# Chang-Tun-Yu/HLS-final-Visual-Odometry

Hardware: AMD Instinct MI355X
Metric: stereo frame-pairs/sec (detect+match), KITTI 1241x376; matches bit-exact (higher is better)
Workload: dtype u8; 1 GPU; KITTI 1241x376 stereo quad-match (prev/curr x L/R), default 50x50 bins; noise=0, gpu_max_hw_queues=4, streams_per_gpu=256, frames_in_hbm=8, parallelism=1x independent stream groups

## Files before the change

### hls-final-visual-odometry_amd/csrc/engine.hip

```cpp
#include "engine.h"

namespace vh_engine {

thread_local std::string t_last_error;

VhMatchArgs Group::role_args() const {
  VhMatchArgs a{};
  a.S = S; a.pair_cur = pairs(); a.rows = S;
  if (seq) {
    a.rows = seq_n;
    a.seq_prev_last = std::max(seq_n_prev - 1, 0);
    a.seq_lo = seq_first == 0 ? 1 : 0;
    a.seq_void = 2 * VH_RING * S;
  }
  return a;
}

int32_t Group::sync_all() {
  VH_HIP(hipStreamSynchronize(stream));
  VH_HIP(hipStreamSynchronize(match_stream));
  VH_HIP(hipStreamSynchronize(post_stream));
  VH_HIP(hipStreamSynchronize(down_stream));
  for (int k = 0; k < kVoteStreams; k++) if (vote_stream[k]) VH_HIP(hipStreamSynchronize(vote_stream[k]));
  if (sparse) { const int32_t rs = sparse->sync_all(); if (rs) return rs; }
// ... 93 lines not shown

  sets = VhSets{};
  sets.cap = cap;
  sets.binsize = p.match_binsize;
  sets.inv_binsize = p.match_binsize > 32768 ? 0u : (uint32_t)(((1ull << 32) + p.match_binsize - 1) / p.match_binsize);
  sets.ubn = (dims[0] + p.match_binsize - 1) / p.match_binsize;
  sets.vbn = (dims[1] + p.match_binsize - 1) / p.match_binsize;
  sets.nbins = 4 * sets.ubn * sets.vbn;
  sets.max_tiles = cap / VH_TILE_Q + 5;
  sets.W = dims[0]; sets.H = dims[1];
  {
    const int32_t blk = g.scale * (g.n + 1);
    const int64_t per_axis = (p.match_binsize + blk - 1) / blk + 1;
    sets.stage_cap = (int32_t)std::min<int64_t>(per_axis * per_axis, cap);
  }
  const size_t ns = n_sets();
  if ((rc = dmalloc(&sets.feat, ns * cap * 12, false))) return rc;
  if ((rc = dmalloc(&sets.f_uv, ns * cap, false))) return rc;
  if ((rc = dmalloc(&sets.s_uv, ns * cap, false))) return rc;
  if ((rc = dmalloc(&sets.s_idx, ns * cap, false))) return rc;
  if ((rc = dmalloc(&sets.s_desc, ns * cap * 8, false))) return rc;
  if ((rc = dmalloc(&sets.bin_start, ns * (sets.nbins + 1), true))) return rc;
  if ((rc = dmalloc(&sets.hist, ns * sets.nbins, true))) return rc;
  if ((rc = dmalloc(&sets.cursor, ns * sets.nbins, true))) return rc;
  if ((rc = dmalloc(&sets.tmp_idx, ns * cap, false))) return rc;
  if ((rc = dmalloc(&sets.stage, ns * (size_t)sets.nbins * sets.stage_cap, false))) return rc;
  if ((rc = dmalloc(&sets.count, ns, true))) return rc;
  const size_t nrow = 4 * (size_t)dims[1];
  if ((rc = dmalloc(&sets.row_start, ns * (nrow + 1), true))) return rc;
  if ((rc = dmalloc(&sets.row_hist, ns * nrow, true))) return rc;
  if ((rc = dmalloc(&sets.row_cursor, ns * nrow, true))) return rc;
  if ((rc = dmalloc(&sets.r_pos, ns * cap, false))) return rc;
  if ((rc = dmalloc(&sets.tiles, ns * sets.max_tiles, false))) return rc;
  if ((rc = dmalloc(&sets.tile_cnt, ns, true))) return rc;
  if ((rc = dmalloc(&sets.check, 4, true))) return rc;
  if ((rc = dmalloc(&det.d_rec, 2 * (size_t)S * std::max(g.nblocks, 1), false))) return rc;
  if ((rc = dmalloc(&det.d_chunk_count, 2 * (size_t)S * g.nchunks, true))) return rc;
  for (int k = 0; k < 2; k++) {
    if ((rc = dmalloc(&mt.d_best2[k], 4 * (size_t)S * cap, false))) return rc;
    if ((rc = dmalloc(&mt.d_chain2[k], 2 * (size_t)S * cap, false))) return rc;
  }
  mt.d_best = mt.d_best2[0]; mt.d_chain = mt.d_chain2[0];
  for (int k = 0; k < 2; k++) {
    if ((rc = dmalloc(&mt.d_mchunk2[k], (size_t)S * ((cap + 255) / 256), true))) return rc;
    VH_HIP(mt.h_out[k].alloc((size_t)S, hipHostMallocMapped));
    memset(mt.h_out[k], 0, sizeof(int4) * (size_t)S);
  }
  if ((rc = dmalloc(&mt.d_redo, 2 * (size_t)S, true))) return rc;
  if ((rc = dmalloc((uint8_t **)&mt.d_matches, (size_t)S * mcap * sizeof(vh_p_match), false))) return rc;
  if ((rc = dmalloc(&mt.d_match_count, (size_t)S, true))) return rc;
  if (serial && (size_t)S * mcap * sizeof(vh_p_match) <= (64u << 20)) {
    VH_HIP(mt.h_matches.alloc((size_t)S * mcap, hipHostMallocMapped));
  }
  if ((rc = dmalloc(&mt.d_overflow, (size_t)S, true))) return rc;
  VH_HIP(mt.h_overflow.alloc((size_t)S, hipHostMallocDefault));
  memset(mt.h_overflow, 0, sizeof(int32_t) * (size_t)S);
  if (p.half_resolution)
    if ((rc = dmalloc(&det.d_half, 2 * (size_t)S * g.bplm * g.Hm, false))) return rc;
  if (p.refinement > 0) {
    vh_refine_setup(rf);
    rf.W = dims[0]; rf.H = dims[1]; rf.bpl = dims[2];
    rf.pitch = round_up(dims[0], 16);
    rf.plane = (int64_t)rf.pitch * dims[1];
    rf.mode = p.refinement == 2 ? 2 : 1;
    const size_t nplanes = 2 * VH_RING * (size_t)S;
    if ((rc = dmalloc(&rf.du, nplanes * rf.plane, false))) return rc;
// ... 212 lines not shown
```

### hls-final-visual-odometry_amd/csrc/engine_api.hip

```cpp
#include "engine.h"

#include <mutex>
#include <thread>

namespace vh_engine {

#define ENTER(gq)                                   \
  if (!(gq)) return VH_ERR_INVALID_ARG;             \
  { hipError_t e_ = hipSetDevice((gq)->device);     \
    if (e_ != hipSuccess) { t_last_error = hipGetErrorString(e_); return VH_ERR_HIP; } }

struct Temp {
  Group *gq = nullptr;
  ~Temp() { if (gq) { (void)gq->sync_all(); delete gq; } }
};
int32_t temp_new(const vh_params *p, int32_t device, int32_t mf, int32_t mm, Temp &t) {
  if (!p) return VH_ERR_INVALID_ARG;
  vh_params q = *p;
  q.refinement = 0;
  return group_new(&q, device, 1, mf, mm, &t.gq);
}

struct EgoWork {
  std::mutex mu;
// ... 525 lines not shown
  return gq->get_features(0, which, out12, cap, n);
}
int32_t vh_host_alloc(int32_t device, size_t bytes, void **out) {
  if (!out || bytes == 0) return VH_ERR_INVALID_ARG;
  *out = nullptr;
  const int32_t rc = select_device(device);
  if (rc) return rc;
  VH_HIP(hipHostMalloc(out, bytes, hipHostMallocDefault));
  return VH_OK;
}
int32_t vh_host_free(void *ptr) {
  if (!ptr) return VH_OK;
  VH_HIP(hipHostFree(ptr));
  return VH_OK;
}
int32_t vh_synchronize(vh_matcher *m) { return vh_group_synchronize((vh_group *)m); }
int32_t vh_set_stream(vh_matcher *m, void *hip_stream) { return vh_group_set_stream((vh_group *)m, hip_stream); }
int32_t vh_clear_stream(vh_matcher *m) { return vh_group_clear_stream((vh_group *)m); }
int32_t vh_stream_wait_images(vh_matcher *m, void *hip_stream) { return vh_group_stream_wait_images((vh_group *)m, hip_stream); }

#ifdef VH_DEBUG_ROWS
int32_t vh_debug_rows(vh_matcher *m, int32_t which, int32_t *row_start, int32_t *r_pos, int32_t *bin_start) {
  Group *gq = (Group *)m; ENTER(gq);
  const int32_t set = vh_role_set(gq->S, gq->pairs(), 0, which);
  const size_t nrow = 4 * (size_t)gq->dims[1];
  VH_HIP(hipDeviceSynchronize());
  VH_HIP(hipMemcpy(row_start, gq->sets.row_start + (size_t)set * (nrow + 1), sizeof(int32_t) * (nrow + 1), hipMemcpyDeviceToHost));
  VH_HIP(hipMemcpy(r_pos, gq->sets.r_pos + (size_t)set * gq->cap, sizeof(int32_t) * gq->cap, hipMemcpyDeviceToHost));
  VH_HIP(hipMemcpy(bin_start, gq->sets.bin_start + (size_t)set * (gq->sets.nbins + 1), sizeof(int32_t) * (gq->sets.nbins + 1), hipMemcpyDeviceToHost));
  return gq->cap;
}
#endif

void vh_default_ego_params(vh_ego_params *e) {
  if (!e) return;
  memset(e, 0, sizeof(*e));
  e->ransac_iters = 200; e->reweighting = 1; e->inlier_threshold = 2.0;
  e->f = 1; e->cu = 0; e->cv = 0; e->base = 1;
}
int32_t vh_group_estimate_motion(vh_group *g, const vh_ego_params *e, const int32_t *rand3, double *tr, int32_t *ok,
                                 int32_t *n_inliers) {
  Group *gq = (Group *)g; ENTER(gq);
  return gq->estimate_motion(e, rand3, tr, ok, n_inliers);
}
int32_t vh_estimate_motion_stereo(const vh_ego_params *e, int32_t device, int32_t n_sets, const vh_p_match *pm,
                                  const int32_t *offsets, const int32_t *rand3, double *tr, int32_t *ok,
                                  int32_t *n_inliers, int32_t *inliers) {
  if (!e) return VH_ERR_INVALID_ARG;
  return estimate_stateless(device, n_sets, e->ransac_iters, 3, false, pm, offsets, rand3, tr, ok, n_inliers, inliers,
    [&](int64_t cap) { return sizeof(double) * 4 * (size_t)n_sets * (size_t)cap; },
    [&](const vh_p_match *d_pm, const int32_t *d_off, const int32_t *d_rand, uint8_t *d_scr, int64_t cap, double *d_tr, int32_t *d_ok, int32_t *d_inl) {
      vh_launch_ego(*e, n_sets, d_pm, 0, d_off, nullptr, 0, d_rand, (double *)d_scr, cap, d_tr, d_ok, d_ok + n_sets, d_inl, 0, nullptr);
    });
}

int32_t vh_group_post_begin(vh_group *g, int32_t cap_per_stream) {
  Group *gq = (Group *)g; ENTER(gq);
  return gq->post_begin(cap_per_stream);
}
int32_t vh_group_post_finish(vh_group *g, int32_t age, int32_t max_features, float bucket_width, float bucket_height, int32_t host_threads,
                             const vh_ego_params *e, const int32_t *rand3, double *tr, int32_t *ok, int32_t *n_inliers,
                             vh_p_match *bucketed, int32_t cap_per_stream, int32_t *counts, double *host_ms) {
  Group *gq = (Group *)g; ENTER(gq);
  if (host_threads < 1) host_threads = (int32_t)std::max(1u, std::thread::hardware_concurrency());
  return gq->post_finish(age, max_features, bucket_width, bucket_height, host_threads, e, rand3, nullptr, nullptr, tr, ok, n_inliers, bucketed, cap_per_stream, counts, host_ms);
}
// ... 330 lines not shown
```

### hls-final-visual-odometry_amd/csrc/kernels_bin.hip

```cpp
#include "vh_dev.h"
#include <algorithm>

#define VH_SCAN_T 256

namespace {

__device__ __forceinline__ int32_t bin_coord(int32_t x, int32_t binsize, int32_t nb) {
  return min(x / binsize, nb - 1);
}

__device__ __forceinline__ int32_t feature_bin(const int32_t *__restrict__ f, const VhSets &s) {
  const int32_t u = f[0], v = f[1], c = f[3];
  return (c * s.ubn + bin_coord(u, s.binsize, s.ubn)) * s.vbn + bin_coord(v, s.binsize, s.vbn);
}

__global__ void zero_counters_kernel(VhSets s, int32_t set0, int32_t nsets, int32_t *__restrict__ extra, int64_t n_extra) {
  const int64_t nb = (int64_t)nsets * s.nbins, nr = (int64_t)nsets * 4 * s.H;
  const int64_t total = 2 * nb + 2 * nr + nsets + n_extra;
  int32_t *hist = s.hist + (int64_t)set0 * s.nbins, *cur = s.cursor + (int64_t)set0 * s.nbins;
  int32_t *rh = s.row_hist + (int64_t)set0 * 4 * s.H, *rc = s.row_cursor + (int64_t)set0 * 4 * s.H;
  for (int64_t i = (int64_t)blockIdx.x * blockDim.x + threadIdx.x; i < total; i += (int64_t)gridDim.x * blockDim.x) {
    int64_t k = i;
    if (k < nb) { hist[k] = 0; continue; }
    k -= nb;
// ... 31 lines not shown

template <int EPT, class Load, class Emit>
__device__ __forceinline__ int32_t scan_exclusive(int32_t n, int32_t *sWave, Load load, Emit emit) {
  const int32_t tid = threadIdx.x, w = tid >> 6;
  int32_t carry = 0;
  for (int32_t b0 = 0; b0 < n; b0 += EPT * VH_SCAN_T) {
    const int32_t b = b0 + EPT * tid;
    int32_t v[EPT];
    int32_t mine = 0;
#pragma unroll
    for (int32_t k = 0; k < EPT; k++) { v[k] = (b + k < n) ? load(b + k) : 0; mine += v[k]; }
    const int32_t incl = scan_wave_inclusive(mine);
    if ((tid & 63) == 63) sWave[w] = incl;
    __syncthreads();
    int32_t before = 0, total = 0;
#pragma unroll
    for (int32_t k = 0; k < VH_SCAN_T / 64; k++) {
      const int32_t x = sWave[k];
      before += (k < w) ? x : 0;
      total += x;
    }
    int32_t run = carry + before + incl - mine;
#pragma unroll
    for (int32_t k = 0; k < EPT; k++) {
      if (b + k < n) emit(b + k, run, v[k]);
      run += v[k];
    }
    carry += total;
    __syncthreads();
  }
  return carry;
}

__device__ __forceinline__ void make_tiles(const VhSets &s, const int32_t *__restrict__ bs, int32_t set) {
  const int32_t span = s.ubn * s.vbn;
  int32_t tb[5];
  tb[0] = 0;
#pragma unroll
  for (int32_t c = 0; c < 4; c++) tb[c + 1] = tb[c] + (bs[(c + 1) * span] - bs[c * span] + VH_TILE_Q - 1) / VH_TILE_Q;
  int4 *__restrict__ tiles = s.tiles + (int64_t)set * s.max_tiles;
  for (int32_t i = threadIdx.x; i < 4 * s.ubn; i += VH_SCAN_T) {
    const int32_t c = i / s.ubn, col = i - c * s.ubn;
    const int32_t cls0 = bs[c * span], cls1 = bs[(c + 1) * span];
    const int32_t a = bs[(c * s.ubn + col) * s.vbn] - cls0, b = bs[(c * s.ubn + col + 1) * s.vbn] - cls0;
    for (int32_t t = (a + VH_TILE_Q - 1) / VH_TILE_Q; t * VH_TILE_Q < b; t++) {
      const int32_t k0 = cls0 + t * VH_TILE_Q, slot = tb[c] + t;
      if (slot < s.max_tiles) tiles[slot] = make_int4(k0, min(cls1, k0 + VH_TILE_Q), c, col);
    }
  }
  if (threadIdx.x == 0) s.tile_cnt[set] = min(tb[4], s.max_tiles);
}

__global__ void __launch_bounds__(VH_SCAN_T) bin_scan_kernel(VhSets s, int32_t set0) {
  __shared__ int32_t sWave[VH_SCAN_T / 64];
  const int32_t set = set0 + blockIdx.x, tid = threadIdx.x;
  VH_DET_SETPRIO();
  const int32_t *__restrict__ hist = s.hist + (int64_t)set * s.nbins;
  int32_t *__restrict__ bs = s.bin_start + (int64_t)set * (s.nbins + 1);
  const int32_t nfeat = scan_exclusive<4>(s.nbins, sWave, [&](int32_t b) { return hist[b]; },
                                       [&](int32_t b, int32_t prefix, int32_t) { bs[b] = prefix; });
  if (tid == 0) bs[s.nbins] = nfeat;
  __syncthreads();

  make_tiles(s, bs, set);

  const int32_t nrow = 4 * s.H;
  const int32_t *__restrict__ rh = s.row_hist + (int64_t)set * nrow;
  int32_t *__restrict__ rs = s.row_start + (int64_t)set * (nrow + 1);
  const int32_t nrowfeat = scan_exclusive<4>(nrow, sWave, [&](int32_t r) { return rh[r]; },
                                          [&](int32_t r, int32_t prefix, int32_t) { rs[r] = prefix; });
  if (tid == 0) rs[nrow] = nrowfeat;
}

__global__ void bin_fill_kernel(VhSets s, int32_t set0) {
  const int32_t set = set0 + blockIdx.y;
  const int32_t n = min(s.count[set], s.cap);
  for (int32_t i = blockIdx.x * blockDim.x + threadIdx.x; i < n; i += gridDim.x * blockDim.x) {
    const int32_t b = feature_bin(s.feat + ((int64_t)set * s.cap + i) * 12, s);
    const int32_t slot = s.bin_start[(int64_t)set * (s.nbins + 1) + b] + atomicAdd(&s.cursor[(int64_t)set * s.nbins + b], 1);
    s.tmp_idx[(int64_t)set * s.cap + slot] = i;
  }
}

__global__ void __launch_bounds__(256) bin_sort_kernel(VhSets s, int32_t set0, int32_t staged) {
  const int32_t set = set0 + blockIdx.y;
  const int32_t bin = blockIdx.x * 16 + (threadIdx.x >> 4), gl = threadIdx.x & 15;
  if (bin >= s.nbins) return;
  VH_DET_SETPRIO();
  const int32_t *__restrict__ bs = s.bin_start + (int64_t)set * (s.nbins + 1);
  const int32_t p0 = bs[bin], p1 = bs[bin + 1], L = p1 - p0;
  if (L <= 0) return;
#ifdef VH_CHECK
  if (staged && gl == 0) { int32_t len = L; VH_CHECK_RANGE(s, 6, len, 0, s.stage_cap + 1); }
#endif
  const int2 *__restrict__ stg = s.stage + ((int64_t)set * s.nbins + bin) * s.stage_cap - p0;
  const int32_t *__restrict__ tmp = s.tmp_idx + (int64_t)set * s.cap;
  const int32_t *__restrict__ feat = s.feat + (int64_t)set * s.cap * 12;
  int32_t *__restrict__ sidx = s.s_idx + (int64_t)set * s.cap;
  uint32_t *__restrict__ suv = s.s_uv + (int64_t)set * s.cap;
  uint4 *__restrict__ sdesc = (uint4 *)(s.s_desc + (int64_t)set * s.cap * 8);
  const int32_t nrow = 4 * s.H;
  const int32_t *__restrict__ rs = s.row_start + (int64_t)set * (nrow + 1);
  int32_t *__restrict__ rcur = s.row_cursor + (int64_t)set * nrow;
  int32_t *__restrict__ rpos = s.r_pos + (int64_t)set * s.cap;
  for (int32_t e0 = 0; e0 < L; e0 += 16) {
    const int32_t e = e0 + gl;
    int32_t mine = 0x7FFFFFFF, rowrel = 0;
    if (e < L) {
      if (staged) { const int2 m2 = stg[p0 + e]; mine = m2.x; rowrel = m2.y; }
      else mine = tmp[p0 + e];
    }
    uint4 h = make_uint4(0, 0, 0, 0), d0 = h, d1 = h;
    if (e < L) {
      const int32_t *f = feat + (int64_t)mine * 12;
      h = *(const uint4 *)f; d0 = *(const uint4 *)(f + 4); d1 = *(const uint4 *)(f + 8);
    }
    int32_t rank = 0;
    for (int32_t j0 = 0; j0 < L; j0 += 16) {
      const int32_t other = (j0 + gl < L) ? (staged ? stg[p0 + j0 + gl].x : tmp[p0 + j0 + gl]) : 0x7FFFFFFF;
      const int32_t m = min(16, L - j0);
      for (int32_t j = 0; j < m; j++) rank += (__shfl(other, j, 16) < mine) ? 1 : 0;
    }
    if (e < L) {
      const int32_t p = p0 + rank;
      sidx[p] = mine;
      suv[p] = (uint32_t)h.x | ((uint32_t)h.y << 16);
      sdesc[2 * (int64_t)p] = d0;
      sdesc[2 * (int64_t)p + 1] = d1;
      const int32_t row = (int32_t)h.w * s.H + (int32_t)h.y;
      int32_t rp = rs[row] + (staged ? rowrel : atomicAdd(&rcur[row], 1));
      VH_CHECK_RANGE(s, 4, rp, rs[row], rs[row + 1]);
      if (rp < rs[nrow]) rpos[rp] = p;
    }
  }
}

__global__ void ref_index_kernel(VhSets s, int32_t set, int32_t *__restrict__ bs_ref,
                                 int32_t *__restrict__ list_ref) {
  __shared__ int32_t sPos;
  const int32_t *__restrict__ bs = s.bin_start + (int64_t)set * (s.nbins + 1);
  const int32_t *__restrict__ sidx = s.s_idx + (int64_t)set * s.cap;
  if (threadIdx.x == 0) sPos = 0;
  __syncthreads();
  for (int32_t rb = 0; rb < s.nbins; rb++) {
    const int32_t ub = rb % s.ubn, vb = (rb / s.ubn) % s.vbn, c = rb / (s.ubn * s.vbn);
    const int32_t ib = (c * s.ubn + ub) * s.vbn + vb;
    const int32_t p0 = bs[ib], L = bs[ib + 1] - p0, pos = sPos;
    if (threadIdx.x == 0) bs_ref[rb] = pos;
    for (int32_t e = threadIdx.x; e < L; e += blockDim.x) list_ref[pos + e] = sidx[p0 + e];
    __syncthreads();
    if (threadIdx.x == 0) sPos = pos + L;
    __syncthreads();
  }
  if (threadIdx.x == 0) bs_ref[s.nbins] = sPos;
}

}

static int32_t feature_blocks(const VhSets &s) { return std::min(std::max(s.cap / 1024, 8), 256); }

void vh_launch_zero_counters(const VhSets &s, int32_t set0, int32_t nsets, int32_t *extra, int64_t n_extra, hipStream_t st) {
// ... 25 lines not shown
```

### hls-final-visual-odometry_amd/csrc/kernels_match.hip

```cpp
#include "vh_findmatch.h"
#include <algorithm>
#include <cstdlib>
#include <type_traits>

#ifdef VH_FLOW_STATS
__device__ unsigned long long g_flow_stats[12];
extern "C" int32_t vh_debug_flow_stats(unsigned long long *out, int32_t reset) {
  if (hipMemcpyFromSymbol(out, HIP_SYMBOL(g_flow_stats), sizeof(g_flow_stats)) != hipSuccess) return -3;
  if (reset) { unsigned long long z[12] = {0}; if (hipMemcpyToSymbol(HIP_SYMBOL(g_flow_stats), z, sizeof(z)) != hipSuccess) return -3; }
  return 0;
}
#define VH_STAT(k, n) do { if ((threadIdx.x & 63) == 0) atomicAdd(&g_flow_stats[k], (unsigned long long)(n)); } while (0)
#else
#define VH_STAT(k, n) do { } while (0)
#endif

#ifndef VH_MATCH_WAVES
#define VH_MATCH_WAVES 7
#endif
#ifndef VH_SNAKE
#define VH_SNAKE 1
#endif

namespace {

__device__ __forceinline__ int32_t wave_min(int32_t v) {
#pragma unroll
  for (int32_t d = 32; d >= 1; d >>= 1) v = min(v, __shfl_xor(v, d));
  return v;
}
__device__ __forceinline__ int32_t wave_max(int32_t v) {
#pragma unroll
  for (int32_t d = 32; d >= 1; d >>= 1) v = max(v, __shfl_xor(v, d));
  return v;
}

template <bool MAX>
__device__ __forceinline__ int32_t row16_allreduce(int32_t v) {
#define VH_ROW_STEP(CTRL)                                                                   \
  {                                                                                         \
    const int32_t t = __builtin_amdgcn_update_dpp(v, v, CTRL, 0xF, 0xF, false);             \
    v = MAX ? max(v, t) : min(v, t);                                                        \
  }
  VH_ROW_STEP(0x128)
  VH_ROW_STEP(0x124)
  VH_ROW_STEP(0x122)
  VH_ROW_STEP(0x121)
#undef VH_ROW_STEP
  return v;
}

template <class T>
__device__ __forceinline__ T ld_off(const T *base, uint32_t byte_off) { return *(const T *)((const char *)base + byte_off); }
template <class T>
// ... 253 lines not shown
                if (k < g.n) kk[k] = min(kk[k], tested_key_uniform_query(g.qd[k], g.lo2[k], span2, gu, g0, g1, (uint32_t)(pl - pbase)));
            });
        } else {
          const int32_t *__restrict__ crs = s.row_start + (int64_t)cset * (4 * s.H + 1);
          const int32_t *__restrict__ cpos = s.r_pos + (int64_t)cset * s.cap;
          const int32_t x0 = ld_uniform_i32(crs + c * s.H + max(g.vmin - rv, 0));
          const int32_t x1 = ld_uniform_i32(crs + c * s.H + min(g.vmax + rv, s.H - 1) + 1);
          for (int32_t x = x0 + lane; x < x1; x += 64) {
            int32_t cp = cpos[x];
            VH_CHECK_RANGE(s, 3, cp, pbase, pbase + pcnt);
            const uint32_t gu = cuv[cp];
            const uint4 g0 = cdesc[2 * (int64_t)cp], g1 = cdesc[2 * (int64_t)cp + 1];
#pragma unroll
            for (int32_t k = 0; k < VH_REDO_G; k++)
              if (k < g.n) kk[k] = min(kk[k], tested_key_uniform_query(g.qd[k], g.lo2[k], span2, gu, g0, g1, (uint32_t)(cp - pbase)));
          }
        }
#pragma unroll
        for (int32_t k = 0; k < VH_REDO_G; k++)
          if (k < g.n) {
            const uint64_t kf = wave_min_u64(kk[k]);
            int32_t wp = (int32_t)(uint32_t)kf;
            if (kf != ~0ull) VH_CHECK_RANGE(s, 7, wp, 0, pcnt);
            if (lane == g.lane[k]) res = kf == ~0ull ? -1 : pbase + wp;
          }
      }
    }
  }
  if (mine) st_off(tbl, (uint32_t)ld_off(qidx, (uint32_t)qpos * 4u) * 4u, res < 0 ? 0 : ld_off(cidx, (uint32_t)res * 4u));
}

template <int Q, int P, int KM, bool SPEC>
__device__ __forceinline__ void flow_tile(const VhSets &s, const VhMatchArgs &a, int32_t pass, int32_t stream,
                                          int32_t qset, int32_t cset, int32_t q0, int32_t q1, int32_t c, int32_t col0,
                                          int32_t pbase, int32_t pcnt, uint4 *wD, uint32_t *wU, TileOut<Q> &out) {
  constexpr int L = 64 / P;
  static_assert(L == 8 || L == 16, "every 16-lane row must hold the whole tile (row-wise window reduction)");
  constexpr int TRIP = 2 * P;
  const int32_t lane = threadIdx.x & 63, ph = lane / L, l = lane % L;
  const uint32_t *__restrict__ quv = s.s_uv + (int64_t)qset * s.cap;
  const uint4 *__restrict__ qdesc = (const uint4 *)(s.s_desc + (int64_t)qset * s.cap * 8);
  const uint32_t *__restrict__ cuv = s.s_uv + (int64_t)cset * s.cap;
  const uint4 *__restrict__ cdesc = (const uint4 *)(s.s_desc + (int64_t)cset * s.cap * 8);
  const int32_t *__restrict__ cbs = s.bin_start + (int64_t)cset * (s.nbins + 1);
  const int32_t rv = a.pass[pass].flow ? a.radius : a.disp_tol;

  bool (&valid)[Q] = out.valid;
  uint4 (&a0)[Q] = out.a0, (&a1)[Q] = out.a1;
  uint32_t (&uv1)[Q] = out.uv1;
  int32_t v_lo[Q];
  us2 lo2[Q];
  typedef typename KeyT<KM>::type key_t;
  const key_t KNONE = (key_t)~(key_t)0;
  key_t best_key[Q];
  int32_t umin = 0x7FFFFFFF, umax = -1, vmin = 0x7FFFFFFF, vmax = -1;
  int32_t (&qp)[Q] = out.qpos;
#pragma unroll
  for (int32_t qi = 0; qi < Q; qi++) {
    const int32_t q = q0 + L * qi + l;
    valid[qi] = q < q1;
    qp[qi] = valid[qi] ? q : q0;
  }
  {
    const int32_t *__restrict__ qbs = s.bin_start + (int64_t)qset * (s.nbins + 1);
    int32_t colb = col0, j = 0;
    int32_t csv = ld_off(qbs, (uint32_t)((c * s.ubn + min(colb + lane, s.ubn)) * s.vbn) * 4u);
    int32_t A = __builtin_amdgcn_readlane(csv, 0);
    int32_t k[Q];
#pragma unroll
    for (int32_t qi = 0; qi < Q; qi++) k[qi] = qp[qi];
    for (;;) {
      const int32_t B = __builtin_amdgcn_readlane(csv, j + 1);
      if (VH_SNAKE && ((colb + j) & 1)) {
#pragma unroll
        for (int32_t qi = 0; qi < Q; qi++) if (k[qi] >= A && k[qi] < B) qp[qi] = A + B - 1 - k[qi];
      }
      if (B >= q1 || colb + j + 1 >= s.ubn) break;
      A = B;
      if (++j == 63) { colb += 63; j = 0; csv = ld_off(qbs, (uint32_t)((c * s.ubn + min(colb + lane, s.ubn)) * s.vbn) * 4u); }
    }
  }
#pragma unroll
  for (int32_t qi = 0; qi < Q; qi++) {
    const int32_t ql = qp[qi];
    uv1[qi] = ld_off(quv, (uint32_t)ql * 4u);
    a0[qi] = ld_off(qdesc, (uint32_t)ql * 32u); a1[qi] = ld_off(qdesc, (uint32_t)ql * 32u + 16u);
    const int32_t u1 = uv1[qi] & 0xFFFF, v1 = uv1[qi] >> 16;
    v_lo[qi] = v1 - rv;
    lo2[qi] = window_lo2(uv1[qi], a.radius, rv);
    best_key[qi] = KNONE;
    umin = min(umin, u1); umax = max(umax, u1); vmin = min(vmin, v1); vmax = max(vmax, v1);
  }
  umin = __builtin_amdgcn_readfirstlane(row16_allreduce<false>(umin));
  umax = __builtin_amdgcn_readfirstlane(row16_allreduce<true>(umax));
  vmin = __builtin_amdgcn_readfirstlane(row16_allreduce<false>(vmin));
  vmax = __builtin_amdgcn_readfirstlane(row16_allreduce<true>(vmax));
  const VhBins ub = bins_of_interest(s, VhWindow{umin - a.radius, umax + a.radius, vmin - rv, vmax + rv});
  const int32_t UB0 = ub.ub0, UB1 = ub.ub1, VB0 = ub.vb0, VB1 = ub.vb1;
  const us2 span2 = window_span2(a.radius, rv);
  const int32_t ULO_MAX = umax - a.radius, UHI_MIN = umin + a.radius;
  const int32_t VLO_MAX = vmax - rv, VHI_MIN = vmin + rv;
  const int32_t VA0 = SPEC ? 0 : max(VB0, (max(VLO_MAX, 0) + s.binsize - 1) / s.binsize);
  const int32_t VA1 = SPEC ? 0 : min(VB1, (VHI_MIN + 1) / s.binsize - 1);

  auto make_key = [&](auto test, int32_t qi, uint32_t uv2, const uint4 &b0, const uint4 &b1, uint32_t seed) -> key_t {
    constexpr int TEST = decltype(test)::value;
    bool out = false;
    if (TEST == 2) {
      out = outside_window(uv2, lo2[qi], span2);
    } else if (TEST == 1) {
      out = (uint32_t)((int32_t)(uv2 >> 16) - v_lo[qi]) > (uint32_t)(2 * rv);
    }
    const key_t key = sad_key<KM>(a0[qi], a1[qi], b0, b1, seed);
    return (TEST != 0 && out) ? KNONE : key;
  };
  VH_STAT(0, 1); VH_STAT(5, q1 - q0); VH_STAT(6, UB1 - UB0 + 1);
  walk_region_lds<!SPEC>(s, cbs, cuv, cdesc, c, UB0, UB1, VB0, VB1, ULO_MAX, UHI_MIN, VA0, VA1, wD, wU,
    [&](int32_t pc, int32_t p1, int32_t pa0, int32_t pa1, const uint4 *cD, const uint32_t *cU) {
      VH_STAT(1, 1);
      const int32_t mcnt = min(64, p1 - pc);
      const int32_t jend = (mcnt + TRIP - 1) & ~(TRIP - 1);
      const uint4 *rd = cD + ph;
      const uint32_t *ru = cU + ph;
      uint32_t seedA = (uint32_t)(pc - pbase + ph), seedB = seedA + P;
      int32_t j = 0;
      auto trip = [&](auto test, int32_t o) {
        const uint4 dA0 = rd[o], dA1 = rd[o + 64], dB0 = rd[o + P], dB1 = rd[o + 64 + P];
        uint32_t uA = 0, uB = 0;
        if (decltype(test)::value != 0) { uA = ru[o]; uB = ru[o + P]; }
#pragma unroll
        for (int32_t qi = 0; qi < Q; qi++) {
          const key_t kA = make_key(test, qi, uA, dA0, dA1, seedA + (uint32_t)o), kB = make_key(test, qi, uB, dB0, dB1, seedB + (uint32_t)o);
          best_key[qi] = min(min(kA, kB), best_key[qi]);
        }
      };
      auto run = [&](auto test, int32_t jstop) {
        if (jstop > j) VH_STAT(2 + decltype(test)::value, (jstop - j) / TRIP);
        for (; j + 2 * TRIP <= jstop; j += 2 * TRIP) {
          trip(test, 0); trip(test, TRIP);
          rd += 2 * TRIP; ru += 2 * TRIP; seedA += 2 * TRIP; seedB += 2 * TRIP;
        }
        if (j < jstop) {
          trip(test, 0);
          j += TRIP; rd += TRIP; ru += TRIP; seedA += TRIP; seedB += TRIP;
        }
      };
      if (SPEC) {
        run(std::integral_constant<int, 0>{}, jend);
      } else if (pa0 <= pa1) {
        const int32_t ja = min((min(max(pa0 - pc, 0), mcnt) + TRIP - 1) & ~(TRIP - 1), jend);
        const int32_t jb = max(min(max(pa1 - pc, 0), mcnt) & ~(TRIP - 1), ja);
        run(std::integral_constant<int, 1>{}, ja);
        run(std::integral_constant<int, 0>{}, jb);
        run(std::integral_constant<int, 1>{}, jend);
      } else {
        run(std::integral_constant<int, 2>{}, jend);
      }
    });
  out.wp = join_phases<Q, P, KM>(best_key);
}

template <bool SPEC, bool FLOW, class Tile>
__device__ __forceinline__ void search_tile(const VhSets &s, const VhMatchArgs &a, int32_t pass, int32_t stream, int32_t qset, int32_t cset,
                                            int32_t c, int32_t *__restrict__ best, int32_t *__restrict__ redo_count, Tile tile) {
  const int32_t *cbs = s.bin_start + (int64_t)cset * (s.nbins + 1);
  const int32_t pbase = ld_uniform_i32(cbs + c * s.ubn * s.vbn);
  const int32_t pend = ld_uniform_i32(cbs + (c + 1) * s.ubn * s.vbn);
  const int32_t km = key_mode_of(pend - pbase, a.wide_keys);
  TileOut<VH_FLOW_Q> out;
  if (km == KEY_HI16) tile(std::integral_constant<int, KEY_HI16>{}, pbase, pend - pbase, out);
  else if (km == KEY_W19) tile(std::integral_constant<int, KEY_W19>{}, pbase, pend - pbase, out);
  else tile(std::integral_constant<int, KEY_64>{}, pbase, pend - pbase, out);
  finish_tile<VH_FLOW_Q, VH_FLOW_P, SPEC, FLOW>(s, a, pass, stream, qset, cset, c, pbase, pend - pbase, out, best, redo_count);
}

template <bool SPEC>
__device__ __forceinline__ void flow_pass(const VhSets &s, const VhMatchArgs &a, int32_t pass, int32_t stream, int32_t qset,
                                          int32_t cset, uint4 *wD, uint32_t *wU, int32_t *__restrict__ best, int32_t *__restrict__ redo_count) {
  const int32_t ntile = ld_uniform_i32(s.tile_cnt + qset);
  for (int32_t tile = __builtin_amdgcn_readfirstlane(blockIdx.x * 4 + (threadIdx.x >> 6)); tile < ntile;
       tile += gridDim.x * 4) {
    typedef int32_t i32x4 __attribute__((ext_vector_type(4)));
    const i32x4 t = ld_uniform((const i32x4 *)(s.tiles + (int64_t)qset * s.max_tiles + tile));
    const int32_t q0 = __builtin_amdgcn_readfirstlane(t.x), q1 = __builtin_amdgcn_readfirstlane(t.y);
    const int32_t c = __builtin_amdgcn_readfirstlane(t.z), col0 = __builtin_amdgcn_readfirstlane(t.w);
    search_tile<SPEC, true>(s, a, pass, stream, qset, cset, c, best, redo_count,
      [&](auto km, int32_t pbase, int32_t pcnt, TileOut<VH_FLOW_Q> &out) __attribute__((always_inline)) {
        flow_tile<VH_FLOW_Q, VH_FLOW_P, decltype(km)::value, SPEC>(s, a, pass, stream, qset, cset, q0, q1, c, col0, pbase, pcnt, wD, wU, out);
      });
  }
}

template <int Q, int P, int KM, bool SPEC>
__device__ __forceinline__ void rows_tile(const VhSets &s, const VhMatchArgs &a, int32_t pass, int32_t stream, int32_t qset,
                                          int32_t cset, int32_t q0, int32_t q1, int32_t c, int32_t pbase, int32_t pcnt, uint4 *wD,
                                          uint32_t *wU, uint32_t *wV, TileOut<Q> &out) {
  constexpr int L = 64 / P;
  static_assert(L == 8 || L == 16, "every 16-lane row must hold the whole tile");
  constexpr int TRIP = 2 * P;
  const int32_t lane = threadIdx.x & 63, ph = lane / L, l = lane % L;
  const int32_t nrow = 4 * s.H;
  const int32_t *__restrict__ crs = s.row_start + (int64_t)cset * (nrow + 1);
  const int32_t *__restrict__ qpos = s.r_pos + (int64_t)qset * s.cap;
  const uint32_t *__restrict__ quv = s.s_uv + (int64_t)qset * s.cap;
  const uint4 *__restrict__ qdesc = (const uint4 *)(s.s_desc + (int64_t)qset * s.cap * 8);
  const int32_t *__restrict__ cpos = s.r_pos + (int64_t)cset * s.cap;
  const uint32_t *__restrict__ cuv = s.s_uv + (int64_t)cset * s.cap;
  const uint4 *__restrict__ cdesc = (const uint4 *)(s.s_desc + (int64_t)cset * s.cap * 8);

  bool (&valid)[Q] = out.valid;
  uint4 (&a0)[Q] = out.a0, (&a1)[Q] = out.a1;
  uint32_t (&uv1)[Q] = out.uv1;
  int32_t (&qp)[Q] = out.qpos;
  typedef typename KeyT<KM>::type key_t;
  key_t best_key[Q];
  us2 lo2[Q];
  const us2 span2 = window_span2(a.radius, a.disp_tol);
  int32_t vmin = 0x7FFFFFFF, vmax = -1;
#pragma unroll
  for (int32_t qi = 0; qi < Q; qi++) {
    const int32_t q = q0 + L * qi + l;
// ... 118 lines not shown
```

### hls-final-visual-odometry_amd/csrc/vh_dev.h

```cpp
#ifndef VH_DEV_H
#define VH_DEV_H

#include <hip/hip_runtime.h>
#include <stdint.h>

#define VH_MARGIN 7
#ifndef VH_CHUNK
#define VH_CHUNK 1024
#endif
#define VH_WAVE 64
#ifndef VH_FLOW_Q
#define VH_FLOW_Q 2
#endif
#ifndef VH_FLOW_P
#define VH_FLOW_P 4
#endif
#define VH_TILE_Q (64 * VH_FLOW_Q / VH_FLOW_P)
#define VH_NO_CODE 0xFFFFu
#ifndef VH_DET_PRIO
#define VH_DET_PRIO 1
#endif
#define VH_DET_SETPRIO() do { if (VH_DET_PRIO) __builtin_amdgcn_s_setprio(VH_DET_PRIO); } while (0)
#define VH_CLASS_POS_BITS 19
#define VH_CLASS_POS_MAX ((1 << VH_CLASS_POS_BITS) - 64)
#define VH_MASK_IDX_BITS 24

struct VhGeom {
  int32_t W, H, bpl;
  int32_t Wm, Hm, bplm;
  int32_t scale;
  int32_t n, tau;
  int32_t nbx, nby, nblocks, nchunks;
  int32_t tbx, tby;
  int32_t FW, FH, IW, IH;
  int32_t IWp, FWp;
};

struct VhSets {
  int32_t *feat;
  uint32_t *f_uv;
  uint32_t *s_uv;
  int32_t *s_idx;
  uint32_t *s_desc;
  int32_t *bin_start;
  int32_t *hist;
  int32_t *cursor;
  int32_t *tmp_idx;
  int2 *stage;
  int32_t *count;
  int32_t *row_start;
  int32_t *row_hist;
  int32_t *row_cursor;
  int32_t *r_pos;
  int4 *tiles;
  int32_t *tile_cnt;
  int32_t cap, nbins, ubn, vbn, binsize, max_tiles;
  uint32_t inv_binsize;
  int32_t W, H;
  int32_t stage_cap;
  uint32_t *check;
};

#ifdef VH_CHECK
#define VH_CHECK_RANGE(s_, code_, x_, lo_, hi_)                                          \
  do {                                                                                   \
    if ((x_) < (lo_) || (x_) >= (hi_)) {                                                 \
      if (atomicAdd(&(s_).check[0], 1u) == 0u) {                                         \
        (s_).check[1] = (uint32_t)(code_); (s_).check[2] = (uint32_t)(x_); (s_).check[3] = (uint32_t)(hi_); \
      }                                                                                  \
      (x_) = (lo_) < (hi_) ? (((x_) < (lo_)) ? (lo_) : (hi_) - 1) : (lo_);                \
    }                                                                                    \
  } while (0)
#else
#define VH_CHECK_RANGE(s_, code_, x_, lo_, hi_) do { } while (0)
#endif

struct VhPass {
  int32_t qset;
  int32_t cset;
  int32_t flow;
  int32_t slot;
};

struct VhMatchArgs {
  VhPass pass[4];
  int32_t npass;
  int32_t pair_cur;
// ... 153 lines not shown
```

Measured before the change: 116,900 pairs/s.

## Precompute per-tile query positions and bounding boxes during binning

Tiles now carry their u/v bounding box, and a per-tile array of query positions (with snake reordering already applied) is filled while features are scattered into bins, using atomic min/max. The match kernel then loads these directly instead of walking the column bin starts to undo the snake order and running cross-lane reductions for the bounding box. This moves work from the hot match loop into the bin kernel. In exchange it adds atomics and scattered stores to binning, a larger tile record, and extra memory for the position table. It also adds debug entry points for inspecting tiles.

Result: slower. 68130 pairs/s (-41.7%).

```diff
diff --git a/hls-final-visual-odometry_amd/csrc/engine.hip b/hls-final-visual-odometry_amd/csrc/engine.hip
--- a/hls-final-visual-odometry_amd/csrc/engine.hip
+++ b/hls-final-visual-odometry_amd/csrc/engine.hip
@@ -149,6 +149,7 @@
   if ((rc = dmalloc(&sets.row_cursor, ns * nrow, true))) return rc;
   if ((rc = dmalloc(&sets.r_pos, ns * cap, false))) return rc;
   if ((rc = dmalloc(&sets.tiles, ns * sets.max_tiles, false))) return rc;
+  if ((rc = dmalloc(&sets.tile_qpos, ns * sets.max_tiles * VH_TILE_Q, true))) return rc;
   if ((rc = dmalloc(&sets.tile_cnt, ns, true))) return rc;
   if ((rc = dmalloc(&sets.check, 4, true))) return rc;
   if ((rc = dmalloc(&det.d_rec, 2 * (size_t)S * std::max(g.nblocks, 1), false))) return rc;
diff --git a/hls-final-visual-odometry_amd/csrc/engine_api.hip b/hls-final-visual-odometry_amd/csrc/engine_api.hip
--- a/hls-final-visual-odometry_amd/csrc/engine_api.hip
+++ b/hls-final-visual-odometry_amd/csrc/engine_api.hip
@@ -581,6 +581,37 @@
 }
 #endif
 
+static int32_t debug_tiles(Group *gq, int32_t set, int32_t *info, int32_t *records, int32_t *qpos, int32_t *bin_start, uint32_t *s_uv) {
+  const VhSets &s = gq->sets;
+  VH_HIP(hipDeviceSynchronize());
+  int32_t cnt = 0;
+  VH_HIP(hipMemcpy(&cnt, s.tile_cnt + set, sizeof(int32_t), hipMemcpyDeviceToHost));
+  if (info) { info[0] = s.cap; info[1] = s.max_tiles; info[2] = s.nbins; info[3] = cnt; }
+  if (records) VH_HIP(hipMemcpy(records, s.tiles + (size_t)set * s.max_tiles, sizeof(VhTile) * (size_t)s.max_tiles, hipMemcpyDeviceToHost));
+  if (qpos) VH_HIP(hipMemcpy(qpos, s.tile_qpos + (size_t)set * s.max_tiles * VH_TILE_Q, sizeof(int32_t) * (size_t)s.max_tiles * VH_TILE_Q, hipMemcpyDeviceToHost));
+  if (bin_start) VH_HIP(hipMemcpy(bin_start, s.bin_start + (size_t)set * (s.nbins + 1), sizeof(int32_t) * ((size_t)s.nbins + 1), hipMemcpyDeviceToHost));
+  if (s_uv) VH_HIP(hipMemcpy(s_uv, s.s_uv + (size_t)set * s.cap, sizeof(uint32_t) * (size_t)s.cap, hipMemcpyDeviceToHost));
+  return VH_OK;
+}
+int32_t vh_debug_tiles(vh_group *g, int32_t stream, int32_t which, int32_t *info, int32_t *records, int32_t *qpos, int32_t *bin_start,
+                       uint32_t *s_uv) {
+  Group *gq = (Group *)g; ENTER(gq);
+  if (!gq->allocated) return VH_ERR_STATE;
+  if (stream < 0 || stream >= gq->S || which < 0 || which > 3) return VH_ERR_INVALID_ARG;
+  return debug_tiles(gq, vh_role_set(gq->S, gq->pairs(), stream, which), info, records, qpos, bin_start, s_uv);
+}
+int32_t vh_debug_tiles_of(const vh_params *p, int32_t device, const int32_t dims[3], const int32_t *m, int32_t n, int32_t *info,
+                          int32_t *records, int32_t *qpos, int32_t *bin_start, uint32_t *s_uv) {
+  if (!p || !dims) return VH_ERR_INVALID_ARG;
+  Temp t;
+  int32_t rc;
+  if ((rc = temp_new(p, device, std::max(n, 64), 1, t))) return rc;
+  const int32_t d[3] = {dims[0], dims[1], std::max(dims[2], dims[0])};
+  if ((rc = t.gq->ensure(d))) return rc;
+  if ((rc = t.gq->load_features(VH_SET_1C, m, n))) return rc;
+  return debug_tiles(t.gq, vh_role_set(1, t.gq->pairs(), 0, VH_SET_1C), info, records, qpos, bin_start, s_uv);
+}
+
 void vh_default_ego_params(vh_ego_params *e) {
   if (!e) return;
   memset(e, 0, sizeof(*e));
diff --git a/hls-final-visual-odometry_amd/csrc/kernels_bin.hip b/hls-final-visual-odometry_amd/csrc/kernels_bin.hip
--- a/hls-final-visual-odometry_amd/csrc/kernels_bin.hip
+++ b/hls-final-visual-odometry_amd/csrc/kernels_bin.hip
@@ -87,23 +87,55 @@
   return carry;
 }
 
+
+__device__ __forceinline__ void tile_bases(const VhSets &s, const int32_t *__restrict__ bs, int32_t (&tb)[5]) {
+  const int32_t span = s.ubn * s.vbn;
+  tb[0] = 0;
+#pragma unroll
+  for (int32_t c = 0; c < 4; c++) tb[c + 1] = tb[c] + (bs[(c + 1) * span] - bs[c * span] + VH_TILE_Q - 1) / VH_TILE_Q;
+}
+
 __device__ __forceinline__ void make_tiles(const VhSets &s, const int32_t *__restrict__ bs, int32_t set) {
   const int32_t span = s.ubn * s.vbn;
   int32_t tb[5];
-  tb[0] = 0;
-#pragma unroll
-  for (int32_t c = 0; c < 4; c++) tb[c + 1] = tb[c] + (bs[(c + 1) * span] - bs[c * span] + VH_TILE_Q - 1) / VH_TILE_Q;
-  int4 *__restrict__ tiles = s.tiles + (int64_t)set * s.max_tiles;
+  tile_bases(s, bs, tb);
+  VhTile *__restrict__ tiles = s.tiles + (int64_t)set * s.max_tiles;
   for (int32_t i = threadIdx.x; i < 4 * s.ubn; i += VH_SCAN_T) {
     const int32_t c = i / s.ubn, col = i - c * s.ubn;
     const int32_t cls0 = bs[c * span], cls1 = bs[(c + 1) * span];
     const int32_t a = bs[(c * s.ubn + col) * s.vbn] - cls0, b = bs[(c * s.ubn + col + 1) * s.vbn] - cls0;
     for (int32_t t = (a + VH_TILE_Q - 1) / VH_TILE_Q; t * VH_TILE_Q < b; t++) {
       const int32_t k0 = cls0 + t * VH_TILE_Q, slot = tb[c] + t;
-      if (slot < s.max_tiles) tiles[slot] = make_int4(k0, min(cls1, k0 + VH_TILE_Q), c, col);
+      if (slot < s.max_tiles) tiles[slot] = VhTile{k0, min(cls1, k0 + VH_TILE_Q), c, 0, 0x7FFFFFFF, -1, 0x7FFFFFFF, -1};
     }
   }
   if (threadIdx.x == 0) s.tile_cnt[set] = min(tb[4], s.max_tiles);
+}
+
+struct TileBin {
+  int32_t colA, colB;
+  int32_t cls0, cls1;
+  int32_t tile0;
+  bool odd;
+};
+__device__ __forceinline__ TileBin tile_bin(const VhSets &s, const int32_t *__restrict__ bs, int32_t bin) {
+  const int32_t span = s.ubn * s.vbn, ccol = bin / s.vbn;
+  const int32_t c = (bin >= span) + (bin >= 2 * span) + (bin >= 3 * span);
+  int32_t tb[5];
+  tile_bases(s, bs, tb);
+  return TileBin{bs[ccol * s.vbn], bs[(ccol + 1) * s.vbn], bs[c * span], bs[(c + 1) * span], tb[c], VH_SNAKE && ((ccol - c * s.ubn) & 1)};
+}
+__device__ __forceinline__ void tile_enter(const VhSets &s, int32_t set, const TileBin &tb, int32_t p, int32_t u, int32_t v) {
+  const int32_t k = tb.odd ? tb.colA + tb.colB - 1 - p : p;
+  const int32_t r = k - tb.cls0, t = tb.tile0 + r / VH_TILE_Q, j = r % VH_TILE_Q;
+  if (t >= s.max_tiles) return;
+  int32_t *__restrict__ tq = s.tile_qpos + ((int64_t)set * s.max_tiles + t) * VH_TILE_Q;
+  tq[j] = p;
+  if (j == 0)
+    for (int32_t jj = tb.cls1 - k; jj < VH_TILE_Q; jj++) tq[jj] = p;
+  VhTile *tile = s.tiles + (int64_t)set * s.max_tiles + t;
+  atomicMin(&tile->umin, u); atomicMax(&tile->umax, u);
+  atomicMin(&tile->vmin, v); atomicMax(&tile->vmax, v);
 }
 
 __global__ void __launch_bounds__(VH_SCAN_T) bin_scan_kernel(VhSets s, int32_t set0) {
@@ -158,6 +190,7 @@
   const int32_t *__restrict__ rs = s.row_start + (int64_t)set * (nrow + 1);
   int32_t *__restrict__ rcur = s.row_cursor + (int64_t)set * nrow;
   int32_t *__restrict__ rpos = s.r_pos + (int64_t)set * s.cap;
+  const TileBin tbin = tile_bin(s, bs, bin);
   for (int32_t e0 = 0; e0 < L; e0 += 16) {
     const int32_t e = e0 + gl;
     int32_t mine = 0x7FFFFFFF, rowrel = 0;
@@ -182,6 +215,7 @@
       suv[p] = (uint32_t)h.x | ((uint32_t)h.y << 16);
       sdesc[2 * (int64_t)p] = d0;
       sdesc[2 * (int64_t)p + 1] = d1;
+      tile_enter(s, set, tbin, p, (int32_t)h.x, (int32_t)h.y);
       const int32_t row = (int32_t)h.w * s.H + (int32_t)h.y;
       int32_t rp = rs[row] + (staged ? rowrel : atomicAdd(&rcur[row], 1));
       VH_CHECK_RANGE(s, 4, rp, rs[row], rs[row + 1]);
diff --git a/hls-final-visual-odometry_amd/csrc/kernels_match.hip b/hls-final-visual-odometry_amd/csrc/kernels_match.hip
--- a/hls-final-visual-odometry_amd/csrc/kernels_match.hip
+++ b/hls-final-visual-odometry_amd/csrc/kernels_match.hip
@@ -17,9 +17,6 @@
 
 #ifndef VH_MATCH_WAVES
 #define VH_MATCH_WAVES 7
-#endif
-#ifndef VH_SNAKE
-#define VH_SNAKE 1
 #endif
 
 namespace {
@@ -339,7 +336,7 @@
 
 template <int Q, int P, int KM, bool SPEC>
 __device__ __forceinline__ void flow_tile(const VhSets &s, const VhMatchArgs &a, int32_t pass, int32_t stream,
-                                          int32_t qset, int32_t cset, int32_t q0, int32_t q1, int32_t c, int32_t col0,
+                                          int32_t qset, int32_t cset, const VhTile &t, const int32_t *__restrict__ tq,
                                           int32_t pbase, int32_t pcnt, uint4 *wD, uint32_t *wU, TileOut<Q> &out) {
   constexpr int L = 64 / P;
   static_assert(L == 8 || L == 16, "every 16-lane row must hold the whole tile (row-wise window reduction)");
@@ -360,48 +357,23 @@
   typedef typename KeyT<KM>::type key_t;
   const key_t KNONE = (key_t)~(key_t)0;
   key_t best_key[Q];
-  int32_t umin = 0x7FFFFFFF, umax = -1, vmin = 0x7FFFFFFF, vmax = -1;
   int32_t (&qp)[Q] = out.qpos;
 #pragma unroll
   for (int32_t qi = 0; qi < Q; qi++) {
-    const int32_t q = q0 + L * qi + l;
-    valid[qi] = q < q1;
-    qp[qi] = valid[qi] ? q : q0;
-  }
-  {
-    const int32_t *__restrict__ qbs = s.bin_start + (int64_t)qset * (s.nbins + 1);
-    int32_t colb = col0, j = 0;
-    int32_t csv = ld_off(qbs, (uint32_t)((c * s.ubn + min(colb + lane, s.ubn)) * s.vbn) * 4u);
-    int32_t A = __builtin_amdgcn_readlane(csv, 0);
-    int32_t k[Q];
-#pragma unroll
-    for (int32_t qi = 0; qi < Q; qi++) k[qi] = qp[qi];
-    for (;;) {
-      const int32_t B = __builtin_amdgcn_readlane(csv, j + 1);
-      if (VH_SNAKE && ((colb + j) & 1)) {
-#pragma unroll
-        for (int32_t qi = 0; qi < Q; qi++) if (k[qi] >= A && k[qi] < B) qp[qi] = A + B - 1 - k[qi];
-      }
-      if (B >= q1 || colb + j + 1 >= s.ubn) break;
-      A = B;
-      if (++j == 63) { colb += 63; j = 0; csv = ld_off(qbs, (uint32_t)((c * s.ubn + min(colb + lane, s.ubn)) * s.vbn) * 4u); }
-    }
+    valid[qi] = l < t.q1 - t.q0 - L * qi;
+    qp[qi] = ld_off(tq + L * qi, (uint32_t)l * 4u);
+    VH_CHECK_RANGE(s, 10, qp[qi], 0, s.cap);
   }
 #pragma unroll
   for (int32_t qi = 0; qi < Q; qi++) {
     const int32_t ql = qp[qi];
     uv1[qi] = ld_off(quv, (uint32_t)ql * 4u);
     a0[qi] = ld_off(qdesc, (uint32_t)ql * 32u); a1[qi] = ld_off(qdesc, (uint32_t)ql * 32u + 16u);
-    const int32_t u1 = uv1[qi] & 0xFFFF, v1 = uv1[qi] >> 16;
-    v_lo[qi] = v1 - rv;
+    v_lo[qi] = (int32_t)(uv1[qi] >> 16) - rv;
     lo2[qi] = window_lo2(uv1[qi], a.radius, rv);
     best_key[qi] = KNONE;
-    umin = min(umin, u1); umax = max(umax, u1); vmin = min(vmin, v1); vmax = max(vmax, v1);
-  }
-  umin = __builtin_amdgcn_readfirstlane(row16_allreduce<false>(umin));
-  umax = __builtin_amdgcn_readfirstlane(row16_allreduce<true>(umax));
-  vmin = __builtin_amdgcn_readfirstlane(row16_allreduce<false>(vmin));
-  vmax = __builtin_amdgcn_readfirstlane(row16_allreduce<true>(vmax));
+  }
+  const int32_t c = t.c, umin = t.umin, umax = t.umax, vmin = t.vmin, vmax = t.vmax;
   const VhBins ub = bins_of_interest(s, VhWindow{umin - a.radius, umax + a.radius, vmin - rv, vmax + rv});
   const int32_t UB0 = ub.ub0, UB1 = ub.ub1, VB0 = ub.vb0, VB1 = ub.vb1;
   const us2 span2 = window_span2(a.radius, rv);
@@ -421,7 +393,7 @@
     const key_t key = sad_key<KM>(a0[qi], a1[qi], b0, b1, seed);
     return (TEST != 0 && out) ? KNONE : key;
   };
-  VH_STAT(0, 1); VH_STAT(5, q1 - q0); VH_STAT(6, UB1 - UB0 + 1);
+  VH_STAT(0, 1); VH_STAT(5, t.q1 - t.q0); VH_STAT(6, UB1 - UB0 + 1);
   walk_region_lds<!SPEC>(s, cbs, cuv, cdesc, c, UB0, UB1, VB0, VB1, ULO_MAX, UHI_MIN, VA0, VA1, wD, wU,
     [&](int32_t pc, int32_t p1, int32_t pa0, int32_t pa1, const uint4 *cD, const uint32_t *cU) {
       VH_STAT(1, 1);
@@ -487,13 +459,16 @@
   const int32_t ntile = ld_uniform_i32(s.tile_cnt + qset);
   for (int32_t tile = __builtin_amdgcn_readfirstlane(blockIdx.x * 4 + (threadIdx.x >> 6)); tile < ntile;
        tile += gridDim.x * 4) {
-    typedef int32_t i32x4 __attribute__((ext_vector_type(4)));
-    const i32x4 t = ld_uniform((const i32x4 *)(s.tiles + (int64_t)qset * s.max_tiles + tile));
-    const int32_t q0 = __builtin_amdgcn_readfirstlane(t.x), q1 = __builtin_amdgcn_readfirstlane(t.y);
-    const int32_t c = __builtin_amdgcn_readfirstlane(t.z), col0 = __builtin_amdgcn_readfirstlane(t.w);
-    search_tile<SPEC, true>(s, a, pass, stream, qset, cset, c, best, redo_count,
+    typedef int32_t i32x8 __attribute__((ext_vector_type(8)));
+    const int64_t slot = (int64_t)qset * s.max_tiles + tile;
+    const i32x8 r = ld_uniform((const i32x8 *)(s.tiles + slot));
+    const VhTile t{__builtin_amdgcn_readfirstlane(r[0]), __builtin_amdgcn_readfirstlane(r[1]), __builtin_amdgcn_readfirstlane(r[2]), 0,
+                   __builtin_amdgcn_readfirstlane(r[4]), __builtin_amdgcn_readfirstlane(r[5]), __builtin_amdgcn_readfirstlane(r[6]),
+                   __builtin_amdgcn_readfirstlane(r[7])};
+    const int32_t *__restrict__ tq = s.tile_qpos + slot * VH_TILE_Q;
+    search_tile<SPEC, true>(s, a, pass, stream, qset, cset, t.c, best, redo_count,
       [&](auto km, int32_t pbase, int32_t pcnt, TileOut<VH_FLOW_Q> &out) __attribute__((always_inline)) {
-        flow_tile<VH_FLOW_Q, VH_FLOW_P, decltype(km)::value, SPEC>(s, a, pass, stream, qset, cset, q0, q1, c, col0, pbase, pcnt, wD, wU, out);
+        flow_tile<VH_FLOW_Q, VH_FLOW_P, decltype(km)::value, SPEC>(s, a, pass, stream, qset, cset, t, tq, pbase, pcnt, wD, wU, out);
       });
   }
 }
diff --git a/hls-final-visual-odometry_amd/csrc/vh_dev.h b/hls-final-visual-odometry_amd/csrc/vh_dev.h
--- a/hls-final-visual-odometry_amd/csrc/vh_dev.h
+++ b/hls-final-visual-odometry_amd/csrc/vh_dev.h
@@ -16,6 +16,9 @@
 #define VH_FLOW_P 4
 #endif
 #define VH_TILE_Q (64 * VH_FLOW_Q / VH_FLOW_P)
+#ifndef VH_SNAKE
+#define VH_SNAKE 1
+#endif
 #define VH_NO_CODE 0xFFFFu
 #ifndef VH_DET_PRIO
 #define VH_DET_PRIO 1
@@ -34,6 +37,11 @@
   int32_t tbx, tby;
   int32_t FW, FH, IW, IH;
   int32_t IWp, FWp;
+};
+
+struct VhTile {
+  int32_t q0, q1, c, pad;
+  int32_t umin, umax, vmin, vmax;
 };
 
 struct VhSets {
@@ -52,7 +60,8 @@
   int32_t *row_hist;
   int32_t *row_cursor;
   int32_t *r_pos;
-  int4 *tiles;
+  VhTile *tiles;
+  int32_t *tile_qpos;
   int32_t *tile_cnt;
   int32_t cap, nbins, ubn, vbn, binsize, max_tiles;
   uint32_t inv_binsize;
```
